# AlibabaResearch/efficientteacher

Measured on AMD Instinct MI355X. Metric: SSOD images/sec (teacher+student step) YOLOv5l 640px, higher is better.
Workload: dtype bf16

## Files before the change

efficientteacher_amd/csrc/conv.hip:

```cpp
#include "conv_host.h"

#ifndef ET_S1_NT
#define ET_S1_NT 1
#endif
#ifndef ET_GLDS_SHORTK_WGS
#define ET_GLDS_SHORTK_WGS 4
#endif


__device__ __forceinline__ void tap_lookup_uniform(const GatherGeom& g, int tap, int& dy, int& dx, int& wt) {
    const int ti = g.tapinfo[__builtin_amdgcn_readfirstlane(tap)];
    dy = (int)(signed char)(ti & 0xff);
    dx = (int)(signed char)((ti >> 8) & 0xff);
    wt = (ti >> 16) & 0xff;
}

__device__ __forceinline__ void tile_of_block(const GatherGeom& g, int& bx, int& by) {
    int id = blockIdx.x;
    if (g.nfast) {
        if (g.xcd_swz) {
            const int nb = gridDim.x, q = nb >> 3, r = nb & 7, xcd = id & 7, k = id >> 3;
            id = (xcd < r ? xcd * (q + 1) : r * (q + 1) + (xcd - r) * q) + k;
        }
        bx = id / g.ntn;
// ... 87 lines not shown
    constexpr int TN = BN / WN / 32, WCOLS = BN / WN, CVN = WCOLS / 8;
    const int l31 = lane & 31, hi = lane >> 5;
    const bool bnb = MODE == 1 ? false : ep.bn_y != nullptr;
    __syncthreads();
    float* const r0 = red + (wm * 2) * BN + wn * WCOLS;
    if (bnb) {
        const int scv = lane % CVN;
#pragma unroll
        for (int e = 0; e < 8; ++e)
            for (int m = CVN; m < 64; m <<= 1) { st.bs1[e] += __shfl_xor(st.bs1[e], m); st.bs2[e] += __shfl_xor(st.bs2[e], m); }
        if (lane < CVN) {
#pragma unroll
            for (int e = 0; e < 8; ++e) { r0[scv * 8 + e] = st.bs1[e]; r0[BN + scv * 8 + e] = st.bs2[e]; }
        }
    } else {
#pragma unroll
        for (int tn = 0; tn < TN; ++tn) {
            const float sv = st.ssum[tn] + __shfl_xor(st.ssum[tn], 32);
            const float qv = st.ssq[tn] + __shfl_xor(st.ssq[tn], 32);
            if (hi == 0) { r0[tn * 32 + l31] = sv; r0[BN + tn * 32 + l31] = qv; }
        }
    }
    __syncthreads();
    float* const dst = ep.stats + ((size_t)(blockIdx.x % ET_BN_SHARDS) * 2) * ep.stats_ld + n0;
    for (int i = tid; i < 2 * BN; i += 64 * WM * WN) {
        const int t = i / BN, c = i % BN;
        float v = 0.f;
#pragma unroll
        for (int w = 0; w < WM; ++w) v += red[(w * 2 + t) * BN + c];
        if (n0 + c < g.Cout) unsafeAtomicAdd(dst + (size_t)t * ep.stats_ld + c, v);
    }
}

template <typename T, int BM, int BN, int WM, int WN, int ACT, int SROWS = 32, int MODE = 0, bool DEFER = false, bool EPF = true>
__device__ __forceinline__ void conv_epilogue_act(f32x16 (&acc)[BM / WM / 32][BN / WN / 32], u32x4* lds_raw, T* __restrict__ Y,
                                                  const GatherGeom& g, const Epilogue& ep, int bx, int m0, int n0, int tid,
                                                  int lane, int wm, int wn, EpiSums<BN / WN / 32>& st) {
    constexpr int TM = BM / WM / 32, TN = BN / WN / 32;
    static_assert(SROWS == 32 || SROWS == 16, "slab rows");
    constexpr int NH = 32 / SROWS;
    using L = EpiLds<BM, BN, WM, WN, SROWS>;
    constexpr int WCOLS = L::WCOLS, SLD = L::SLD;
    constexpr int CVN = WCOLS / 8;
    constexpr int RPI = 64 / CVN;
    static_assert(RPI <= SROWS, "a store iteration covers at most one slab");
    const int l31 = lane & 31, hi = lane >> 5;
    const int wave = wm * WN + wn;
    float* const stg = (float*)lds_raw + wave * L::SLAB;
    float (&ssum)[TN] = st.ssum;
    float (&ssq)[TN] = st.ssq;
    float (&bs1)[8] = st.bs1;
    float (&bs2)[8] = st.bs2;
    const bool ident = (g.osy == 1 && g.osx == 1 && g.ooy == 0 && g.oox == 0 && g.QH == g.OH && g.QW == g.OW);
    float csc[TN], cbi[TN];
#pragma unroll
    for (int tn = 0; tn < TN; ++tn) {
        const int co = n0 + wn * WCOLS + tn * 32 + l31;
        const bool cok = co < g.Cout;
        if constexpr (DEFER) {
            csc[tn] = st.cst[co - n0];
            cbi[tn] = st.cst[st.cstride + co - n0];
        } else {
            csc[tn] = (ep.scale && cok) ? ep.scale[co] : 1.0f;
            cbi[tn] = (ep.bias && cok) ? ep.bias[co] : 0.0f;
        }
    }
    const int srow = lane / CVN, scv = lane % CVN;
    const int co = n0 + wn * WCOLS + scv * 8;
    const bool bnb = MODE == 1 ? false : ep.bn_y != nullptr;
    const void* const ep_res = MODE == 1 ? nullptr : ep.res;
    const bool ep_accumulate = MODE == 1 ? false : (bool)ep.accumulate;
    const bool lean = ident && !bnb && ep_res == nullptr && !ep_accumulate && m0 + (wm + 1) * (BM / WM) <= g.M && n0 + BN <= g.Cout;
    float bsc[8], bsh[8];
#pragma unroll
    for (int e = 0; e < 8; ++e) { bsc[e] = 1.f; bsh[e] = 0.f; }
    if (bnb && co + 8 <= g.Cout) {
#pragma unroll
        for (int e = 0; e < 8; ++e) {
            if constexpr (DEFER) { bsc[e] = st.cst[2 * st.cstride + co - n0 + e]; bsh[e] = st.cst[3 * st.cstride + co - n0 + e]; }
            else { bsc[e] = ep.bn_scale[co + e]; bsh[e] = ep.bn_shift[co + e]; }
        }
    }
    auto bn_bwd_sums = [&](const float (&dz8)[8], const float (&y8)[8]) {
        auto body = [&](auto act_tag) {
            constexpr int BACT = decltype(act_tag)::value;
#pragma unroll
            for (int e = 0; e < 8; ++e) {
                const float u = y8[e] * bsc[e] + bsh[e];
                float gact = 1.f;
                if constexpr (BACT == ACT_SILU) { const float sg = __builtin_amdgcn_rcpf(1.0f + __expf(-u)); gact = sg * (1.0f + u * (1.0f - sg)); }
                else if constexpr (BACT == ACT_RELU) gact = u > 0.f ? 1.f : 0.f;
                const float du = dz8[e] * gact;
                bs1[e] += du;
                bs2[e] += du * y8[e];
            }
        };
        if (ep.bn_act == ACT_SILU) body(std::integral_constant<int, ACT_SILU>{});
        else if (ep.bn_act == ACT_RELU) body(std::integral_constant<int, ACT_RELU>{});
        else body(std::integral_constant<int, ACT_NONE>{});
    };
    constexpr int NIT = SROWS / RPI;
    constexpr bool PF = EPF && sizeof(T) == 2 && MODE == 0;
    const bool pf_on = PF && !lean && (ep_res != nullptr || ep_accumulate || bnb);
    const bool pf_a_is_res = ep_res != nullptr;
    u32x4 pf_a[NIT], pf_b[NIT];
    auto pix_of = [&](int p) -> long long {
        if (ident) return p;
        const uint32_t t1 = fdiv((uint32_t)p, g.dQW), qx = p - t1 * g.QW;
        const uint32_t n = fdiv(t1, g.dQH), qy = t1 - n * g.QH;
        return ((long long)n * g.OH + (qy * g.osy + g.ooy)) * g.OW + (qx * g.osx + g.oox);
    };
#pragma unroll
    for (int tmh = 0; tmh < TM * NH; ++tmh) {
        const int tm = tmh / NH, hoff = (tmh % NH) * SROWS;
        if constexpr (PF) {
            if (pf_on) {
#pragma unroll
                for (int it = 0; it < NIT; ++it) {
                    const int p = m0 + wm * (BM / WM) + tm * 32 + hoff + it * RPI + srow;
                    if (p < g.M && co + 8 <= g.Cout) {
                        const long long pix = pix_of(p);
                        if (pf_a_is_res) pf_a[it] = *(const u32x4*)((const T*)ep_res + pix * ep.ldr + co);
                        else if (ep_accumulate) pf_a[it] = *(const u32x4*)(Y + pix * g.ldy + co);
                        if (bnb) pf_b[it] = *(const u32x4*)((const T*)ep.bn_y + pix * ep.ld_bn + co);
                    }
                }
            }
        }
#pragma unroll
        for (int rr = 0; rr < 16 / NH; ++rr) {
            const int r = (tmh % NH) * (16 / NH) + rr;
            const int row = (rr & 3) + 8 * (rr >> 2) + 4 * hi;
#pragma unroll
            for (int tn = 0; tn < TN; ++tn) {
                float v = acc[tm][tn][r];
                ssum[tn] += v;
                ssq[tn] += v * v;
                v = v * csc[tn] + cbi[tn];
                if constexpr (ACT == ACT_SILU) v = v * __builtin_amdgcn_rcpf(1.0f + __expf(-v));
                else if constexpr (ACT == ACT_RELU) v = fmaxf(v, 0.f);
                stg[row * SLD + tn * 32 + l31] = v;
            }
        }
        __builtin_amdgcn_s_waitcnt(0xC07F);
        __builtin_amdgcn_wave_barrier();
        if constexpr (sizeof(T) == 2) {
            if (lean) {
#pragma unroll
                for (int it = 0; it < SROWS / RPI; ++it) {
                    const int row = it * RPI + srow;
                    const long long p = m0 + wm * (BM / WM) + tm * 32 + hoff + row;
                    const float4 a = *(const float4*)(stg + row * SLD + scv * 8);
                    const float4 b = *(const float4*)(stg + row * SLD + scv * 8 + 4);
                    *(u32x4*)(Y + p * g.ldy + co) = mk4(et_lp<T>::pack(a.x, a.y), et_lp<T>::pack(a.z, a.w), et_lp<T>::pack(b.x, b.y), et_lp<T>::pack(b.z, b.w));
                }
                __builtin_amdgcn_s_waitcnt(0xC07F);
                __builtin_amdgcn_wave_barrier();
                continue;
            }
        }
#pragma unroll
        for (int it = 0; it < SROWS / RPI; ++it) {
            const int row = it * RPI + srow;
            const int p = m0 + wm * (BM / WM) + tm * 32 + hoff + row;
            if (p < g.M && co < g.Cout) {
                const long long pix = pix_of(p);
                float v[8];
                const float4 a = *(const float4*)(stg + row * SLD + scv * 8);
                const float4 b = *(const float4*)(stg + row * SLD + scv * 8 + 4);
                v[0] = a.x; v[1] = a.y; v[2] = a.z; v[3] = a.w; v[4] = b.x; v[5] = b.y; v[6] = b.z; v[7] = b.w;
                T* yp = Y + pix * g.ldy + co;
                if (co + 8 <= g.Cout) {
                    if constexpr (sizeof(T) == 2) {
                        if (ep_res) {
                            u32x4 rr;
// ... 31 lines not shown
                        }
                    } else {
                        if (ep_res) {
                            const float* rp = (const float*)ep_res + pix * ep.ldr + co;
                            const float4 r0 = *(const float4*)rp, r1 = *(const float4*)(rp + 4);
                            v[0] += r0.x; v[1] += r0.y; v[2] += r0.z; v[3] += r0.w; v[4] += r1.x; v[5] += r1.y; v[6] += r1.z; v[7] += r1.w;
                        }
                        if (ep_accumulate) {
                            const float4 r0 = *(const float4*)yp, r1 = *(const float4*)((const float*)yp + 4);
                            v[0] += r0.x; v[1] += r0.y; v[2] += r0.z; v[3] += r0.w; v[4] += r1.x; v[5] += r1.y; v[6] += r1.z; v[7] += r1.w;
                        }
                        *(float4*)yp = make_float4(v[0], v[1], v[2], v[3]);
                        *(float4*)((float*)yp + 4) = make_float4(v[4], v[5], v[6], v[7]);
                        if (bnb) {
                            const float* bp = (const float*)ep.bn_y + pix * ep.ld_bn + co;
                            const float4 y0 = *(const float4*)bp, y1 = *(const float4*)(bp + 4);
                            const float yv8[8] = {y0.x, y0.y, y0.z, y0.w, y1.x, y1.y, y1.z, y1.w};
                            bn_bwd_sums(v, yv8);
                        }
                    }
                } else {
                    for (int e = 0; e < 8 && co + e < g.Cout; ++e) {
                        float x = v[e];
                        if (ep_res) x += et_elem<T>::ld(((const T*)ep_res)[pix * ep.ldr + co + e]);
                        if (ep_accumulate) x += et_elem<T>::ld(yp[e]);
                        yp[e] = et_elem<T>::st(x);
                    }
                }
            }
        }
        __builtin_amdgcn_s_waitcnt(0xC07F);
        __builtin_amdgcn_wave_barrier();
    }
    if constexpr (!DEFER) {
        if (ep.stats) {
            constexpr int RPW = (BM / WM) / 64;
            static_assert((BM / WM) % 64 == 0, "wave tiles are whole 64-row blocks");
            if (ep.stats_ld) conv_stats_add_sharded_wg<BN, WN, WM, MODE>(st, g, ep, tid, lane, wm, wn, (float*)lds_raw, n0);
            else conv_epilogue_write_stats<BN, WN, MODE>(st, g, ep, n0, lane, wn, (m0 + wm * (BM / WM)) / 64, RPW - 1, (g.M + 63) / 64);
        }
    }
}

template <typename T, int BM, int BN, int WM, int WN, int SROWS = 32, int MODE = 0, bool DEFER = false, bool EPF = true>
__device__ __forceinline__ void conv_epilogue(f32x16 (&acc)[BM / WM / 32][BN / WN / 32], u32x4* lds_raw, T* __restrict__ Y,
                                              const GatherGeom& g, const Epilogue& ep, int bx, int m0, int n0, int tid,
                                              int lane, int wm, int wn, EpiSums<BN / WN / 32>& st) {
    if (ep.act == ACT_SILU) conv_epilogue_act<T, BM, BN, WM, WN, ACT_SILU, SROWS, MODE, DEFER, EPF>(acc, lds_raw, Y, g, ep, bx, m0, n0, tid, lane, wm, wn, st);
    else if (ep.act == ACT_RELU) conv_epilogue_act<T, BM, BN, WM, WN, ACT_RELU, SROWS, MODE, DEFER, EPF>(acc, lds_raw, Y, g, ep, bx, m0, n0, tid, lane, wm, wn, st);
    else conv_epilogue_act<T, BM, BN, WM, WN, ACT_NONE, SROWS, MODE, DEFER, EPF>(acc, lds_raw, Y, g, ep, bx, m0, n0, tid, lane, wm, wn, st);
}
template <typename T, int BM, int BN, int WM, int WN, bool EPF = true>
__device__ __forceinline__ void conv_epilogue(f32x16 (&acc)[BM / WM / 32][BN / WN / 32], u32x4* lds_raw, T* __restrict__ Y,
                                              const GatherGeom& g, const Epilogue& ep, int bx, int m0, int n0, int tid,
                                              int lane, int wm, int wn) {
    EpiSums<BN / WN / 32> st;
    st.clear();
    conv_epilogue<T, BM, BN, WM, WN, 32, 0, false, EPF>(acc, lds_raw, Y, g, ep, bx, m0, n0, tid, lane, wm, wn, st);
}

template <typename T, int BM, int BN, int WM, int WN, int BKV, bool UTAP>
__global__ __launch_bounds__(256) void conv_gemm_kernel(const T* __restrict__ X, const T* __restrict__ W,
                                                        T* __restrict__ Y, GatherGeom g, Epilogue ep) {
    constexpr int VEC = et_elem<T>::VEC;
    constexpr int TM = BM / WM / 32, TN = BN / WN / 32;
    constexpr int RPT = 256 / BKV;
    constexpr int RA = BM / RPT, RB = BN / RPT;
    constexpr int STAGE_VEC = (BM + BN) * BKV;
    constexpr int EPI_VEC = EpiLds<BM, BN, WM, WN>::VEC16;
    constexpr int LDS_VEC = 2 * STAGE_VEC > EPI_VEC ? 2 * STAGE_VEC : EPI_VEC;
    __shared__ __attribute__((aligned(16))) u32x4 lds_raw[LDS_VEC];
    u32x4* const lds0 = lds_raw;
    u32x4* const lds1 = lds_raw + STAGE_VEC;

    const int tid = threadIdx.x, lane = tid & 63, wave = tid >> 6;
    const int wm = wave / WN, wn = wave % WN;
    int bx, by;
    tile_of_block(g, bx, by);
    const int m0 = bx * BM, n0 = by * BN;
    const int lvec = tid % BKV, lrow = tid / BKV;

    int a_off[RA], a_iy[RA], a_ix[RA];
    bool a_ok[RA];
#pragma unroll
    for (int j = 0; j < RA; ++j) {
        const int p = m0 + lrow + j * RPT;
// ... 286 lines not shown
        const int P = P0 - 1 + rho;
        const uint32_t Pp = P < 0 ? 0 : P;
        const uint32_t yg = fdiv(Pp, g.dW1), xp = Pp - yg * W1;
        const uint32_t pix = yg * g.QW + xp;
        a_ok[q] = rho < CAP && P >= 0 && (int)xp < g.QW && pix < (uint32_t)g.M;
        const uint32_t ygc = a_ok[q] ? yg : 0;
        a_iy[q] = ygc - fdiv(ygc, g.dQH) * g.QH;
        a_off[q] = (a_ok[q] ? pix : 0) * g.ldx;
        a_lv[q] = lvec ^ lds_swz<BKV>(rho);
    }
    const int rowstep = g.IW * g.ldx;
    unsigned a_nokm = 0u;
    et_rsrc rsX, rsW;
    if constexpr (BUF) {
        rsX = et_make_rsrc((const char*)X - (size_t)rowstep * sizeof(T), (unsigned)(((size_t)g.N * g.IH * g.IW * g.ldx + rowstep) * sizeof(T)));
        rsW = et_make_rsrc(W, (unsigned)((size_t)g.Cout * g.TT * g.Cin * sizeof(T)));
#pragma unroll
        for (int q = 0; q < RA; ++q) {
            a_nokm |= ((a_iy[q] > 0 ? 0u : 1u) | (a_iy[q] + 1 < g.IH ? 0u : 4u)) << (3 * q);
            a_off[q] = a_ok[q] ? (int)((a_off[q] + a_lv[q] * VEC) * (int)sizeof(T)) : (int)0x80000000;
        }
    }
    int b_off[RB], b_lv[RB];
    bool b_ok[RB];
#pragma unroll
    for (int q = 0; q < RB; ++q) {
        const int rl = lrow + q * RPT;
        const int co = n0 + rl;
        b_ok[q] = co < g.Cout;
        b_off[q] = (b_ok[q] ? co : 0) * g.TT * g.Cin;
        b_lv[q] = lvec ^ lds_swz<BKV>(rl);
        if constexpr (BUF) b_off[q] = (int)((co * g.TT * g.Cin + b_lv[q] * VEC) * (int)sizeof(T));
    }
    int abase[TM][3];
#pragma unroll
    for (int tm = 0; tm < TM; ++tm) {
        const uint32_t p = m0 + wm * (BM / WM) + tm * 32 + (lane & 31);
        const uint32_t yg = fdiv(p, g.dQW);
        const int r0 = (int)(yg * W1 + (p - yg * g.QW)) - P0;
#pragma unroll
        for (int sft = 0; sft < 3; ++sft) abase[tm][sft] = ((r0 + sft) * BKV + ((lane >> 5) ^ lds_swz<BKV>(r0 + sft))) * 16;
    }

    f32x16 acc[TM][TN];
#pragma unroll
    for (int tm = 0; tm < TM; ++tm)
#pragma unroll
        for (int tn = 0; tn < TN; ++tn)
#pragma unroll
            for (int r = 0; r < 16; ++r) acc[tm][tn][r] = 0.f;

    const int sgn = g.dy[0] < 0 ? 1 : -1;
    auto stage_a = [&](u32x4* dst, int j, int cv_c) {
        u32x4* const wbase = dst + wave * 64;
        const int dy = sgn * (j - 1);
        const int roff = dy * g.IW * g.ldx + cv_c * VEC;
#pragma unroll
        for (int q = 0; q < RA; ++q) {
            if (q == RAF && wave >= XW) continue;
            if constexpr (BUF) {
                const unsigned bad = (a_nokm >> (3 * q + 1 + dy)) & 1u;
                et_bufdma16(rsX, (bad << 31) | (unsigned)a_off[q], (unsigned)(((dy + 1) * rowstep + cv_c * VEC) * (int)sizeof(T)), wbase + q * NT);
            } else {
                const bool ok = a_ok[q] && (unsigned)(a_iy[q] + dy) < (unsigned)g.IH;
                const T* src = ok ? X + (a_off[q] + roff + a_lv[q] * VEC) : ZERO;
                et_glds16(src, wbase + q * NT);
            }
        }
    };
    auto stage_b = [&](u32x4* dst, int tap, int cv_c) {
        u32x4* const wbase = dst + wave * 64;
        const int woff = tap * g.Cin + cv_c * VEC;
#pragma unroll
        for (int q = 0; q < RB; ++q) {
            if constexpr (BUF) {
                et_bufdma16(rsW, (unsigned)b_off[q], (unsigned)(woff * (int)sizeof(T)), wbase + q * NT);
            } else {
                const T* src = b_ok[q] ? W + (b_off[q] + woff + b_lv[q] * VEC) : ZERO;
                et_glds16(src, wbase + q * NT);
            }
        }
    };
    auto mma_step = [&](const u32x4* __restrict__ sa, const u32x4* __restrict__ sb, auto shift_tag) {
        constexpr int SFT = decltype(shift_tag)::value;
        const int l31 = lane & 31, gh = lane >> 5;
        u32x4 af[2][TM], bf[2][TN];
        auto fetch = [&](int kk, int set) {
#pragma unroll
            for (int tm = 0; tm < TM; ++tm) af[set][tm] = *(const u32x4*)((const char*)sa + (abase[tm][SFT] ^ (kk * 32)));
#pragma unroll
            for (int tn = 0; tn < TN; ++tn) {
                const int r = wn * (BN / WN) + tn * 32 + l31;
                bf[set][tn] = sb[r * BKV + ((kk * 2 + gh) ^ lds_swz<BKV>(r))];
            }
        };
        fetch(0, 0);
#pragma unroll
        for (int kk = 0; kk < BKV / 2; ++kk) {
            const int cur = kk & 1;
            if (kk + 1 < BKV / 2) {
                fetch(kk + 1, cur ^ 1);
                __builtin_amdgcn_sched_barrier(0);
            }
#pragma unroll
            for (int tm = 0; tm < TM; ++tm)
#pragma unroll
                for (int tn = 0; tn < TN; ++tn)
                    acc[tm][tn] = et_mfma32<T>(af[cur][tm], bf[cur][tn], acc[tm][tn]);
        }
    };

    const int nunits = 3 * (g.CV / BKV);
    stage_a(slotA, 0, 0);
    stage_b(slotB, sgn > 0 ? 0 : 2, 0);
    int j = 0, cv_u = 0, bs = 0;
#pragma unroll 1
    for (int u = 0; u < nunits; ++u) {
        const bool more_units = u + 1 < nunits;
        int nj = j + 1, ncv = cv_u;
        if (nj == 3) { nj = 0; ncv += BKV; }
        const u32x4* const sa = slotA + (u & 1) * A_VEC;
        auto step = [&](auto ktag) {
            constexpr int k = decltype(ktag)::value;
            if (k == 1 && more_units) {
                if (wave < XW) et_wait_vmem_le_lds_read_done<RA>(); else et_wait_vmem_le_lds_read_done<RAF>();
            } else {
                et_wait_vmem_lds_read_done();
            }
            __builtin_amdgcn_s_barrier();
            constexpr int kn = k < 2 ? k + 1 : 0;
            if (k < 2 || more_units) stage_b(slotB + (bs ^ 1) * B_VEC, (k < 2 ? j : nj) * 3 + (sgn > 0 ? kn : 2 - kn), k < 2 ? cv_u : ncv);
            if (k == 0 && more_units) stage_a(slotA + ((u + 1) & 1) * A_VEC, nj, ncv);
            mma_step(sa, slotB + bs * B_VEC, ktag);
            bs ^= 1;
        };
        step(std::integral_constant<int, 0>{});
        step(std::integral_constant<int, 1>{});
        step(std::integral_constant<int, 2>{});
        j = nj; cv_u = ncv;
    }
    __syncthreads();
// ... 33 lines not shown
    tile_of_block(g, bx, by);
    const int m0 = bx * BM, n0 = by * BN;
    const int lvec = tid & 7, lrow = tid >> 3;
    const int lv = lvec ^ lds_swz<BKV>(lrow);

    int a_off[2][2], a_iy[2][2], a_ix[2][2];
    unsigned a_okm = 0u, b_okm = 0u;
#pragma unroll
    for (int i = 0; i < 2; ++i)
#pragma unroll
        for (int jj = 0; jj < 2; ++jj) {
            const int p = m0 + jj * 128 + i * 64 + lrow;
            const bool ok = p < g.M;
            const uint32_t pp = ok ? p : 0;
            const uint32_t t1 = fdiv(pp, g.dQW), qx = pp - t1 * g.QW;
            const uint32_t n = fdiv(t1, g.dQH), qy = t1 - n * g.QH;
            a_iy[i][jj] = qy * g.isy;
            a_ix[i][jj] = qx * g.isx;
            a_off[i][jj] = ((n * g.IH + a_iy[i][jj]) * g.IW + a_ix[i][jj]) * g.ldx;
            a_okm |= ok ? (1u << (i * 2 + jj)) : 0u;
        }
    int b_off[2][2];
#pragma unroll
    for (int j = 0; j < 2; ++j)
#pragma unroll
        for (int jj = 0; jj < 2; ++jj) {
            const int r = jj * 64 + lrow;
            const int co = n0 + (r >> 5) * 64 + j * 32 + (r & 31);
            const bool ok = co < g.Cout;
            b_off[j][jj] = (ok ? co : 0) * g.TT * g.Cin;
            b_okm |= ok ? (1u << (j * 2 + jj)) : 0u;
        }

    f32x16 acc[4][2];
#pragma unroll
    for (int tm = 0; tm < 4; ++tm)
#pragma unroll
        for (int tn = 0; tn < 2; ++tn)
#pragma unroll
            for (int r = 0; r < 16; ++r) acc[tm][tn][r] = 0.f;

    const int nchunks = g.KV / BKV;
    int tap_u = 0, cv_u = 0;
    int ti_cur = g.tapinfo[0];
    int udy = 0, udx = 0, uwt = 0;
#define ET_PP_DECODE()                                                   \
    do {                                                                 \
        udy = (int)(signed char)(ti_cur & 0xff);                         \
        udx = (int)(signed char)((ti_cur >> 8) & 0xff);                  \
        uwt = (ti_cur >> 16) & 0xff;                                     \
    } while (0)
#define ET_PP_ADVANCE()                                                  \
    do {                                                                 \
        const int t2_ = tap_u + 1, c2_ = cv_u + BKV;                     \
        const bool wt_ = t2_ >= g.T, wc_ = c2_ >= g.CV;                  \
        const int ta_ = wt_ ? 0 : t2_, ca_ = wt_ ? c2_ : cv_u;           \
        const int cb_ = wc_ ? 0 : c2_, tb_ = wc_ ? t2_ : tap_u;          \
        tap_u = g.tap_inner ? ta_ : tb_;                                 \
        cv_u = g.tap_inner ? ca_ : cb_;                                  \
        ti_cur = g.tapinfo[__builtin_amdgcn_readfirstlane(tap_u < g.T ? tap_u : 0)]; \
    } while (0)
    auto stage_piece = [&](int k, int buf, int jj) {
        u32x4* const wbase = lds_raw + (2 * k + buf) * HALF_VEC + wave * 64;
        if (k < 2) {
            const int i = k;
            const int doff = (udy * g.IW + udx) * g.ldx + (cv_u + lv) * VEC;
            const bool ok = (bool)((a_okm >> (i * 2 + jj)) & 1u) & ((unsigned)(a_iy[i][jj] + udy) < (unsigned)g.IH) &
                            ((unsigned)(a_ix[i][jj] + udx) < (unsigned)g.IW);
            et_glds16(ok ? X + (a_off[i][jj] + doff) : ZERO, wbase + jj * 512);
        } else {
            const int j = k - 2;
            const int woff = uwt * g.Cin + (cv_u + lv) * VEC;
            const bool ok = (b_okm >> (j * 2 + jj)) & 1u;
            et_glds16(ok ? W + (b_off[j][jj] + woff) : ZERO, wbase + jj * 512);
        }
    };
    auto stage_a = [&](int i, int buf) { stage_piece(i, buf, 0); stage_piece(i, buf, 1); };
    auto stage_b = [&](int j, int buf) { stage_piece(2 + j, buf, 0); stage_piece(2 + j, buf, 1); };

    const int l31 = lane & 31, gk = lane >> 5;
    u32x4 af[2][4], bf[4];
    auto load_a = [&](int i, int buf) {
        const u32x4* sm = lds_raw + (2 * i + buf) * HALF_VEC;
#pragma unroll
        for (int t = 0; t < 2; ++t) {
            const int r = wm * 64 + t * 32 + l31;
#pragma unroll
            for (int kk = 0; kk < 4; ++kk) af[t][kk] = sm[r * BKV + ((kk * 2 + gk) ^ lds_swz<BKV>(r))];
        }
    };
    auto load_b = [&](int j, int buf) {
        const u32x4* sm = lds_raw + (2 * (2 + j) + buf) * HALF_VEC;
        const int r = wn * 32 + l31;
#pragma unroll
        for (int kk = 0; kk < 4; ++kk) bf[kk] = sm[r * BKV + ((kk * 2 + gk) ^ lds_swz<BKV>(r))];
    };
    auto mfma8 = [&](int i, int j, int sk, int sb) {
        __builtin_amdgcn_s_setprio(1);
        __builtin_amdgcn_sched_barrier(0);
#pragma unroll
        for (int kk = 0; kk < 4; ++kk)
#pragma unroll
            for (int t = 0; t < 2; ++t) {
                acc[2 * i + t][j] = et_mfma32<T>(af[t][kk], bf[kk], acc[2 * i + t][j]);
                const int n = kk * 2 + t;
                if (sk >= 0 && (n == 1 || n == 4)) {
                    __builtin_amdgcn_sched_barrier(0);
                    stage_piece(sk, sb, n == 1 ? 0 : 1);
                    __builtin_amdgcn_sched_barrier(0);
                }
            }
        __builtin_amdgcn_sched_barrier(0);
        __builtin_amdgcn_s_setprio(0);
    };

    ET_PP_DECODE();
    stage_a(0, 0); stage_b(0, 0); stage_b(1, 0); stage_a(1, 0);
    ET_PP_ADVANCE();
    et_wait_vmem();
    __builtin_amdgcn_s_barrier();
#define ET_PP_BAR() __builtin_amdgcn_s_barrier()
#define ET_PP_WAIT(n) et_wait_vmem_le_pp<n>()
    if (wm == 1) __builtin_amdgcn_s_barrier();

    auto chunk = [&](int buf, auto last_tag) {
        constexpr bool LAST = decltype(last_tag)::value;
        const int nb = buf ^ 1;
        if constexpr (!LAST) ET_PP_DECODE();
        load_a(0, buf); load_b(0, buf);
        ET_PP_WAIT(2);
        ET_PP_BAR();
        mfma8(0, 0, LAST ? -1 : 0, nb);
        ET_PP_BAR();
        load_b(1, buf);
        if constexpr (LAST) ET_PP_WAIT(0); else ET_PP_WAIT(2);
        ET_PP_BAR();
        mfma8(0, 1, LAST ? -1 : 2, nb);
        ET_PP_BAR();
        load_a(1, buf);
        ET_PP_BAR();
        mfma8(1, 1, LAST ? -1 : 3, nb);
        ET_PP_BAR();
        load_b(0, buf);
        if constexpr (!LAST) ET_PP_WAIT(2);
// ... 45 lines not shown
    const int P0 = (int)(yg0 * W1 + ((uint32_t)m0 - yg0 * g.QW));

    int a_off[NPIECE];
    unsigned a_okm = 0u, b_okm = 0u;
#pragma unroll
    for (int q = 0; q < NPIECE; ++q) {
        const int P = P0 - 1 + q * 64 + lrow;
        const uint32_t Pp = P < 0 ? 0 : P;
        const uint32_t yg = fdiv(Pp, g.dW1), xp = Pp - yg * W1;
        const uint32_t pix = yg * g.QW + xp;
        const bool ok = P >= 0 && (int)xp < g.QW && pix < (uint32_t)g.M;
        const uint32_t ygc = ok ? yg : 0;
        const int iy = ygc - fdiv(ygc, g.dQH) * g.QH;
        a_off[q] = (ok ? pix : 0) * g.ldx;
        a_okm |= ok ? ((iy > 0 ? 1u : 0u) | 2u | (iy + 1 < g.IH ? 4u : 0u)) << (3 * q) : 0u;
        if constexpr (BUF) a_off[q] = ok ? (int)((a_off[q] + lv * VEC) * (int)sizeof(T)) : (int)0x80000000;
    }
    const unsigned a_nokm = ~a_okm;
    const int co0 = n0 + (lrow >> 5) * 64 + (lrow & 31);
    const int wrow = g.TT * g.Cin;
    const int b_off0 = co0 * wrow;
    const int rowstep = g.IW * g.ldx;
    et_rsrc rsX, rsW;
    unsigned voffB = 0;
    if constexpr (BUF) {
        rsX = et_make_rsrc((const char*)X - (size_t)rowstep * sizeof(T), (unsigned)(((size_t)g.N * g.IH * g.IW * g.ldx + rowstep) * sizeof(T)));
        rsW = et_make_rsrc(W, (unsigned)((size_t)g.Cout * wrow * sizeof(T)));
        voffB = (unsigned)((b_off0 + lv * VEC) * (int)sizeof(T));
    }
#pragma unroll
    for (int j = 0; j < 2; ++j)
#pragma unroll
        for (int jj = 0; jj < 2; ++jj) b_okm |= (co0 + jj * 128 + j * 32 < g.Cout) ? (1u << (j * 2 + jj)) : 0u;
    const int l31 = lane & 31, gk = lane >> 5;
    int abase[2][2][3];
#pragma unroll
    for (int i = 0; i < 2; ++i)
#pragma unroll
        for (int t = 0; t < 2; ++t) {
            const uint32_t p = m0 + wm * 128 + i * 64 + t * 32 + l31;
            const uint32_t yg = fdiv(p, g.dQW);
            const int r0 = (int)(yg * W1 + (p - yg * g.QW)) - P0;
#pragma unroll
            for (int sft = 0; sft < 3; ++sft) abase[i][t][sft] = ((r0 + sft) * BKV + (gk ^ lds_swz<BKV>(r0 + sft))) * 16;
        }

    f32x16 acc[4][2];
#pragma unroll
    for (int tm = 0; tm < 4; ++tm)
#pragma unroll
        for (int tn = 0; tn < 2; ++tn)
#pragma unroll
            for (int r = 0; r < 16; ++r) acc[tm][tn][r] = 0.f;

    const int sgn = g.dy[0] < 0 ? 1 : -1;
    auto stage_a_piece = [&](int q, int ub, int j, int cv) {
        u32x4* const wbase = slotA + ub * A_VEC + q * 512 + wave * 64;
        const int dy = sgn * (j - 1);
        if constexpr (BUF) {
            const unsigned bad = (a_nokm >> (3 * q + 1 + dy)) & 1u;
            et_bufdma16(rsX, (bad << 31) | (unsigned)a_off[q], (unsigned)(((dy + 1) * rowstep + cv * VEC) * (int)sizeof(T)), wbase);
        } else {
            const bool ok = (a_okm >> (3 * q + 1 + dy)) & 1u;
            et_glds16(ok ? X + (a_off[q] + dy * g.IW * g.ldx + (cv + lv) * VEC) : ZERO, wbase);
        }
    };
    auto stage_b_piece = [&](int j, int b, int jj, int tap, int cv) {
        u32x4* const wbase = slotB + (2 * j + b) * HALF_VEC + wave * 64;
        if constexpr (BUF) {
            et_bufdma16(rsW, voffB, (unsigned)(((jj * 128 + j * 32) * wrow + tap * g.Cin + cv * VEC) * (int)sizeof(T)), wbase + jj * 512);
        } else {
            const bool ok = (b_okm >> (j * 2 + jj)) & 1u;
            et_glds16(ok ? W + (b_off0 + (jj * 128 + j * 32) * wrow + tap * g.Cin + (cv + lv) * VEC) : ZERO, wbase + jj * 512);
        }
    };

    u32x4 af[2][4], bf[4];
    auto load_a = [&](int i, int ub, auto shift_tag) {
        constexpr int SFT = decltype(shift_tag)::value;
        const char* sm = (const char*)(slotA + ub * A_VEC);
#pragma unroll
        for (int t = 0; t < 2; ++t)
#pragma unroll
            for (int kk = 0; kk < 4; ++kk) af[t][kk] = *(const u32x4*)(sm + (abase[i][t][SFT] ^ (kk * 32)));
    };
    auto load_b = [&](int j, int b) {
        const u32x4* sm = slotB + (2 * j + b) * HALF_VEC;
        const int r = wn * 32 + l31;
#pragma unroll
        for (int kk = 0; kk < 4; ++kk) bf[kk] = sm[r * BKV + ((kk * 2 + gk) ^ lds_swz<BKV>(r))];
    };
    auto mfma8 = [&](int i, int j, auto&& piece0, auto&& piece1) {
        __builtin_amdgcn_s_setprio(1);
        __builtin_amdgcn_sched_barrier(0);
#pragma unroll
        for (int kk = 0; kk < 4; ++kk)
#pragma unroll
            for (int t = 0; t < 2; ++t) {
                acc[2 * i + t][j] = et_mfma32<T>(af[t][kk], bf[kk], acc[2 * i + t][j]);
                const int n = kk * 2 + t;
                if (n == 1) { __builtin_amdgcn_sched_barrier(0); piece0(); __builtin_amdgcn_sched_barrier(0); }
                if (n == 4) { __builtin_amdgcn_sched_barrier(0); piece1(); __builtin_amdgcn_sched_barrier(0); }
            }
        __builtin_amdgcn_sched_barrier(0);
        __builtin_amdgcn_s_setprio(0);
    };
    auto nothing = [] {};

    const int nunits = 3 * (g.CV / BKV);
#pragma unroll
    for (int q = 0; q < NPIECE; ++q) stage_a_piece(q, 0, 0, 0);
#pragma unroll
    for (int j = 0; j < 2; ++j) { stage_b_piece(j, 0, 0, sgn > 0 ? 0 : 2, 0); stage_b_piece(j, 0, 1, sgn > 0 ? 0 : 2, 0); }
    et_wait_vmem();
    __builtin_amdgcn_s_barrier();
#define ET_PP_BAR() __builtin_amdgcn_s_barrier()
#define ET_PP_WAIT(n) et_wait_vmem_le_pp<n>()
    if (wm == 1) __builtin_amdgcn_s_barrier();

    int jrow = 0, cv_u = 0, bbuf = 0;
#pragma unroll 1
    for (int u = 0; u < nunits; ++u) {
        const bool more = u + 1 < nunits;
        int nj = jrow + 1, ncv = cv_u;
        if (nj == 3) { nj = 0; ncv += BKV; }
        const int ub = u & 1, nub = ub ^ 1;
        auto chunk = [&](auto ktag) {
            constexpr int k = decltype(ktag)::value;
            const bool stage_b = k < 2 || more;
            const int kn = k < 2 ? k + 1 : 0;
            const int ntap = (k < 2 ? jrow : nj) * 3 + (sgn > 0 ? kn : 2 - kn), nbcv = k < 2 ? cv_u : ncv;
            const int nb = bbuf ^ 1;
            const std::integral_constant<int, k> shift{};
            load_a(0, ub, shift); load_b(0, bbuf);
            if (k > 0 && more) ET_PP_WAIT(1); else ET_PP_WAIT(0);
            ET_PP_BAR();
// ... 266 lines not shown
```

efficientteacher_amd/csrc/conv_device.h:

```cpp
#pragma once
#include "et_device.h"
#include "../../include/et_hip.h"
#include <stdlib.h>
#include <stdio.h>
#include <string.h>
#include <type_traits>

typedef __attribute__((ext_vector_type(16))) float f32x16;
typedef __attribute__((ext_vector_type(8))) __bf16 bf16x8;
typedef __attribute__((ext_vector_type(8))) _Float16 f16x8;
typedef __attribute__((ext_vector_type(4))) unsigned int u32x4;
typedef short s16x4 __attribute__((ext_vector_type(4)));
typedef short s16x8 __attribute__((ext_vector_type(8)));
__device__ __forceinline__ u32x4 mk4(unsigned a, unsigned b, unsigned c, unsigned d) { u32x4 v = {a, b, c, d}; return v; }
__device__ __forceinline__ void et_pin_loaded(u32x4& v) {
#if defined(__HIP_DEVICE_COMPILE__)
    asm volatile("" : "+v"(v));
#endif
}

template <typename T, typename V> __device__ __forceinline__ f32x16 et_mfma32(const V a, const V b, const f32x16 c) {
    static_assert(sizeof(V) == 16, "8 x 16-bit operands");
    if constexpr (std::is_same<T, et_f16>::value)
        return __builtin_amdgcn_mfma_f32_32x32x16_f16(__builtin_bit_cast(f16x8, a), __builtin_bit_cast(f16x8, b), c, 0, 0, 0);
    else
        return __builtin_amdgcn_mfma_f32_32x32x16_bf16(__builtin_bit_cast(bf16x8, a), __builtin_bit_cast(bf16x8, b), c, 0, 0, 0);
}

#define CONV_MAX_TAPS 36
#define RS_A_ROWS(BM) ((BM) + 16)
#define PPRS_ROWS 320

struct FastDiv {
    uint32_t magic, shift, d;
};
static FastDiv make_fastdiv(uint32_t d) {
    FastDiv f;
    if (d == 0) d = 1;
    f.d = d;
    uint32_t s = 0;
    while ((1ull << s) < d) ++s;
    f.shift = s;
    f.magic = (uint32_t)((((1ull << 32) * ((1ull << s) - d)) / d) + 1);
    return f;
}
__device__ __forceinline__ uint32_t fdiv(uint32_t n, const FastDiv& f) {
    return (__umulhi(n, f.magic) + n) >> f.shift;
}

struct GatherGeom {
    int N, IH, IW, Cin, ldx;
    int QH, QW, M;
    int OH, OW, Cout, ldy;
    int isy, isx;
    int osy, osx, ooy, oox;
    int T, TT;
    int CV, KV;
    int tap_inner;
    int xcd_swz;
// ... 128 lines not shown
```

Measured before the change: 1321.

## Switch conv kernels from 32x32x16 to 16x16x32 MFMA with matching epilogue

```diff
diff --git a/efficientteacher_amd/csrc/conv.hip b/efficientteacher_amd/csrc/conv.hip
--- a/efficientteacher_amd/csrc/conv.hip
+++ b/efficientteacher_amd/csrc/conv.hip
@@ -143,12 +143,15 @@
     }
 }
 
-template <typename T, int BM, int BN, int WM, int WN, int ACT, int SROWS = 32, int MODE = 0, bool DEFER = false, bool EPF = true>
-__device__ __forceinline__ void conv_epilogue_act(f32x16 (&acc)[BM / WM / 32][BN / WN / 32], u32x4* lds_raw, T* __restrict__ Y,
+template <typename T, int BM, int BN, int WM, int WN, int ACT, int SROWS = 32, int MODE = 0, bool DEFER = false, bool EPF = true, typename ACC>
+__device__ __forceinline__ void conv_epilogue_act(ACC& acc, u32x4* lds_raw, T* __restrict__ Y,
                                                   const GatherGeom& g, const Epilogue& ep, int bx, int m0, int n0, int tid,
                                                   int lane, int wm, int wn, EpiSums<BN / WN / 32>& st) {
     constexpr int TM = BM / WM / 32, TN = BN / WN / 32;
-    static_assert(SROWS == 32 || SROWS == 16, "slab rows");
+    constexpr bool M16 = std::is_same<ACC, f32x4[TM][TN][2][2]>::value;
+    static_assert(M16 || std::is_same<ACC, f32x16[TM][TN]>::value, "accumulator form");
+    constexpr int NCI = M16 ? 2 : 1;
+    static_assert(SROWS == 32 || (SROWS == 16 && !M16), "slab rows");
     constexpr int NH = 32 / SROWS;
     using L = EpiLds<BM, BN, WM, WN, SROWS>;
     constexpr int WCOLS = L::WCOLS, SLD = L::SLD;
@@ -163,19 +166,24 @@
     float (&bs1)[8] = st.bs1;
     float (&bs2)[8] = st.bs2;
     const bool ident = (g.osy == 1 && g.osx == 1 && g.ooy == 0 && g.oox == 0 && g.QH == g.OH && g.QW == g.OW);
-    float csc[TN], cbi[TN];
-#pragma unroll
-    for (int tn = 0; tn < TN; ++tn) {
-        const int co = n0 + wn * WCOLS + tn * 32 + l31;
-        const bool cok = co < g.Cout;
-        if constexpr (DEFER) {
-            csc[tn] = st.cst[co - n0];
-            cbi[tn] = st.cst[st.cstride + co - n0];
-        } else {
-            csc[tn] = (ep.scale && cok) ? ep.scale[co] : 1.0f;
-            cbi[tn] = (ep.bias && cok) ? ep.bias[co] : 0.0f;
-        }
-    }
+    const int lcol = M16 ? (lane & 15) : l31;
+    float csc[TN][NCI], cbi[TN][NCI];
+    float s16[TN][NCI], q16[TN][NCI];
+#pragma unroll
+    for (int tn = 0; tn < TN; ++tn)
+#pragma unroll
+        for (int ci = 0; ci < NCI; ++ci) {
+            const int co = n0 + wn * WCOLS + tn * 32 + ci * 16 + lcol;
+            const bool cok = co < g.Cout;
+            if constexpr (DEFER) {
+                csc[tn][ci] = st.cst[co - n0];
+                cbi[tn][ci] = st.cst[st.cstride + co - n0];
+            } else {
+                csc[tn][ci] = (ep.scale && cok) ? ep.scale[co] : 1.0f;
+                cbi[tn][ci] = (ep.bias && cok) ? ep.bias[co] : 0.0f;
+            }
+            s16[tn][ci] = 0.f; q16[tn][ci] = 0.f;
+        }
     const int srow = lane / CVN, scv = lane % CVN;
     const int co = n0 + wn * WCOLS + scv * 8;
     const bool bnb = MODE == 1 ? false : ep.bn_y != nullptr;
@@ -239,19 +247,28 @@
             }
         }
 #pragma unroll
-        for (int rr = 0; rr < 16 / NH; ++rr) {
+        for (int rr = 0; rr < (M16 ? 8 : 16) / NH; ++rr) {
             const int r = (tmh % NH) * (16 / NH) + rr;
-            const int row = (rr & 3) + 8 * (rr >> 2) + 4 * hi;
-#pragma unroll
-            for (int tn = 0; tn < TN; ++tn) {
-                float v = acc[tm][tn][r];
-                ssum[tn] += v;
-                ssq[tn] += v * v;
-                v = v * csc[tn] + cbi[tn];
-                if constexpr (ACT == ACT_SILU) v = v * __builtin_amdgcn_rcpf(1.0f + __expf(-v));
-                else if constexpr (ACT == ACT_RELU) v = fmaxf(v, 0.f);
-                stg[row * SLD + tn * 32 + l31] = v;
-            }
+            const int row = M16 ? 16 * (rr >> 2) + 4 * (lane >> 4) + (rr & 3) : (rr & 3) + 8 * (rr >> 2) + 4 * hi;
+#pragma unroll
+            for (int tn = 0; tn < TN; ++tn)
+#pragma unroll
+                for (int ci = 0; ci < NCI; ++ci) {
+                    float v;
+                    if constexpr (M16) {
+                        v = acc[tm][tn][rr >> 2][ci][rr & 3];
+                        s16[tn][ci] += v;
+                        q16[tn][ci] += v * v;
+                    } else {
+                        v = acc[tm][tn][r];
+                        ssum[tn] += v;
+                        ssq[tn] += v * v;
+                    }
+                    v = v * csc[tn][ci] + cbi[tn][ci];
+                    if constexpr (ACT == ACT_SILU) v = v * __builtin_amdgcn_rcpf(1.0f + __expf(-v));
+                    else if constexpr (ACT == ACT_RELU) v = fmaxf(v, 0.f);
+                    stg[row * SLD + tn * 32 + ci * 16 + lcol] = v;
+                }
         }
         __builtin_amdgcn_s_waitcnt(0xC07F);
         __builtin_amdgcn_wave_barrier();
@@ -349,6 +366,14 @@
         __builtin_amdgcn_s_waitcnt(0xC07F);
         __builtin_amdgcn_wave_barrier();
     }
+    if constexpr (M16) {
+        const bool up = (lane >> 4) & 1;
+#pragma unroll
+        for (int tn = 0; tn < TN; ++tn) {
+            ssum[tn] += (up ? s16[tn][1] : s16[tn][0]) + __shfl_xor(up ? s16[tn][0] : s16[tn][1], 16);
+            ssq[tn] += (up ? q16[tn][1] : q16[tn][0]) + __shfl_xor(up ? q16[tn][0] : q16[tn][1], 16);
+        }
+    }
     if constexpr (!DEFER) {
         if (ep.stats) {
             constexpr int RPW = (BM / WM) / 64;
@@ -359,16 +384,16 @@
     }
 }
 
-template <typename T, int BM, int BN, int WM, int WN, int SROWS = 32, int MODE = 0, bool DEFER = false, bool EPF = true>
-__device__ __forceinline__ void conv_epilogue(f32x16 (&acc)[BM / WM / 32][BN / WN / 32], u32x4* lds_raw, T* __restrict__ Y,
+template <typename T, int BM, int BN, int WM, int WN, int SROWS = 32, int MODE = 0, bool DEFER = false, bool EPF = true, typename ACC>
+__device__ __forceinline__ void conv_epilogue(ACC& acc, u32x4* lds_raw, T* __restrict__ Y,
                                               const GatherGeom& g, const Epilogue& ep, int bx, int m0, int n0, int tid,
                                               int lane, int wm, int wn, EpiSums<BN / WN / 32>& st) {
     if (ep.act == ACT_SILU) conv_epilogue_act<T, BM, BN, WM, WN, ACT_SILU, SROWS, MODE, DEFER, EPF>(acc, lds_raw, Y, g, ep, bx, m0, n0, tid, lane, wm, wn, st);
     else if (ep.act == ACT_RELU) conv_epilogue_act<T, BM, BN, WM, WN, ACT_RELU, SROWS, MODE, DEFER, EPF>(acc, lds_raw, Y, g, ep, bx, m0, n0, tid, lane, wm, wn, st);
     else conv_epilogue_act<T, BM, BN, WM, WN, ACT_NONE, SROWS, MODE, DEFER, EPF>(acc, lds_raw, Y, g, ep, bx, m0, n0, tid, lane, wm, wn, st);
 }
-template <typename T, int BM, int BN, int WM, int WN, bool EPF = true>
-__device__ __forceinline__ void conv_epilogue(f32x16 (&acc)[BM / WM / 32][BN / WN / 32], u32x4* lds_raw, T* __restrict__ Y,
+template <typename T, int BM, int BN, int WM, int WN, bool EPF = true, typename ACC>
+__device__ __forceinline__ void conv_epilogue(ACC& acc, u32x4* lds_raw, T* __restrict__ Y,
                                               const GatherGeom& g, const Epilogue& ep, int bx, int m0, int n0, int tid,
                                               int lane, int wm, int wn) {
     EpiSums<BN / WN / 32> st;
@@ -721,23 +746,25 @@
         b_lv[q] = lvec ^ lds_swz<BKV>(rl);
         if constexpr (BUF) b_off[q] = (int)((co * g.TT * g.Cin + b_lv[q] * VEC) * (int)sizeof(T));
     }
-    int abase[TM][3];
-#pragma unroll
-    for (int tm = 0; tm < TM; ++tm) {
-        const uint32_t p = m0 + wm * (BM / WM) + tm * 32 + (lane & 31);
+    int abase[2 * TM][3];
+#pragma unroll
+    for (int ts = 0; ts < 2 * TM; ++ts) {
+        const uint32_t p = m0 + wm * (BM / WM) + ts * 16 + (lane & 15);
         const uint32_t yg = fdiv(p, g.dQW);
         const int r0 = (int)(yg * W1 + (p - yg * g.QW)) - P0;
 #pragma unroll
-        for (int sft = 0; sft < 3; ++sft) abase[tm][sft] = ((r0 + sft) * BKV + ((lane >> 5) ^ lds_swz<BKV>(r0 + sft))) * 16;
-    }
-
-    f32x16 acc[TM][TN];
+        for (int sft = 0; sft < 3; ++sft) abase[ts][sft] = ((r0 + sft) * BKV + ((lane >> 4) ^ lds_swz<BKV>(r0 + sft))) * 16;
+    }
+
+    f32x4 acc[TM][TN][2][2];
 #pragma unroll
     for (int tm = 0; tm < TM; ++tm)
 #pragma unroll
         for (int tn = 0; tn < TN; ++tn)
 #pragma unroll
-            for (int r = 0; r < 16; ++r) acc[tm][tn][r] = 0.f;
+            for (int q = 0; q < 4; ++q)
+#pragma unroll
+                for (int r = 0; r < 4; ++r) acc[tm][tn][q >> 1][q & 1][r] = 0.f;
 
     const int sgn = g.dy[0] < 0 ? 1 : -1;
     auto stage_a = [&](u32x4* dst, int j, int cv_c) {
@@ -772,30 +799,38 @@
     };
     auto mma_step = [&](const u32x4* __restrict__ sa, const u32x4* __restrict__ sb, auto shift_tag) {
         constexpr int SFT = decltype(shift_tag)::value;
-        const int l31 = lane & 31, gh = lane >> 5;
-        u32x4 af[2][TM], bf[2][TN];
-        auto fetch = [&](int kk, int set) {
-#pragma unroll
-            for (int tm = 0; tm < TM; ++tm) af[set][tm] = *(const u32x4*)((const char*)sa + (abase[tm][SFT] ^ (kk * 32)));
-#pragma unroll
-            for (int tn = 0; tn < TN; ++tn) {
-                const int r = wn * (BN / WN) + tn * 32 + l31;
-                bf[set][tn] = sb[r * BKV + ((kk * 2 + gh) ^ lds_swz<BKV>(r))];
-            }
+        const int l15 = lane & 15, gq = lane >> 4;
+        u32x4 af[2][TM], bf[2][TN][2];
+        auto fetch_a = [&](int stg) {
+#pragma unroll
+            for (int tm = 0; tm < TM; ++tm) af[stg & 1][tm] = *(const u32x4*)((const char*)sa + (abase[2 * tm + (stg & 1)][SFT] ^ ((stg >> 1) * 64)));
         };
-        fetch(0, 0);
-#pragma unroll
-        for (int kk = 0; kk < BKV / 2; ++kk) {
-            const int cur = kk & 1;
-            if (kk + 1 < BKV / 2) {
-                fetch(kk + 1, cur ^ 1);
+        auto fetch_b = [&](int kk) {
+#pragma unroll
+            for (int tn = 0; tn < TN; ++tn)
+#pragma unroll
+                for (int ci = 0; ci < 2; ++ci) {
+                    const int r = wn * (BN / WN) + tn * 32 + ci * 16 + l15;
+                    bf[kk & 1][tn][ci] = sb[r * BKV + ((kk * 4 + gq) ^ lds_swz<BKV>(r))];
+                }
+        };
+        fetch_a(0);
+        fetch_b(0);
+#pragma unroll
+        for (int stg = 0; stg < BKV / 2; ++stg) {
+            const int kk = stg >> 1, ri = stg & 1;
+            if (stg + 1 < BKV / 2) {
+                fetch_a(stg + 1);
+                if (ri == 1) fetch_b(kk + 1);
                 __builtin_amdgcn_sched_barrier(0);
             }
 #pragma unroll
             for (int tm = 0; tm < TM; ++tm)
 #pragma unroll
                 for (int tn = 0; tn < TN; ++tn)
-                    acc[tm][tn] = et_mfma32<T>(af[cur][tm], bf[cur][tn], acc[tm][tn]);
+#pragma unroll
+                    for (int ci = 0; ci < 2; ++ci)
+                        acc[tm][tn][ri][ci] = et_mfma16<T>(af[ri][tm], bf[kk & 1][tn][ci], acc[tm][tn][ri][ci]);
         }
     };
 
@@ -895,13 +930,15 @@
             b_okm |= ok ? (1u << (j * 2 + jj)) : 0u;
         }
 
-    f32x16 acc[4][2];
+    f32x4 acc[4][2][2][2];
 #pragma unroll
     for (int tm = 0; tm < 4; ++tm)
 #pragma unroll
         for (int tn = 0; tn < 2; ++tn)
 #pragma unroll
-            for (int r = 0; r < 16; ++r) acc[tm][tn][r] = 0.f;
+            for (int q = 0; q < 4; ++q)
+#pragma unroll
+                for (int r = 0; r < 4; ++r) acc[tm][tn][q >> 1][q & 1][r] = 0.f;
 
     const int nchunks = g.KV / BKV;
     int tap_u = 0, cv_u = 0;
@@ -941,38 +978,43 @@
     auto stage_a = [&](int i, int buf) { stage_piece(i, buf, 0); stage_piece(i, buf, 1); };
     auto stage_b = [&](int j, int buf) { stage_piece(2 + j, buf, 0); stage_piece(2 + j, buf, 1); };
 
-    const int l31 = lane & 31, gk = lane >> 5;
-    u32x4 af[2][4], bf[4];
+    const int l15 = lane & 15, gk = lane >> 4;
+    u32x4 af[4][2], bf[2][2];
     auto load_a = [&](int i, int buf) {
         const u32x4* sm = lds_raw + (2 * i + buf) * HALF_VEC;
 #pragma unroll
-        for (int t = 0; t < 2; ++t) {
-            const int r = wm * 64 + t * 32 + l31;
-#pragma unroll
-            for (int kk = 0; kk < 4; ++kk) af[t][kk] = sm[r * BKV + ((kk * 2 + gk) ^ lds_swz<BKV>(r))];
+        for (int ts = 0; ts < 4; ++ts) {
+            const int r = wm * 64 + ts * 16 + l15;
+#pragma unroll
+            for (int kk = 0; kk < 2; ++kk) af[ts][kk] = sm[r * BKV + ((kk * 4 + gk) ^ lds_swz<BKV>(r))];
         }
     };
     auto load_b = [&](int j, int buf) {
         const u32x4* sm = lds_raw + (2 * (2 + j) + buf) * HALF_VEC;
-        const int r = wn * 32 + l31;
-#pragma unroll
-        for (int kk = 0; kk < 4; ++kk) bf[kk] = sm[r * BKV + ((kk * 2 + gk) ^ lds_swz<BKV>(r))];
+#pragma unroll
+        for (int ci = 0; ci < 2; ++ci) {
+            const int r = wn * 32 + ci * 16 + l15;
+#pragma unroll
+            for (int kk = 0; kk < 2; ++kk) bf[ci][kk] = sm[r * BKV + ((kk * 4 + gk) ^ lds_swz<BKV>(r))];
+        }
     };
     auto mfma8 = [&](int i, int j, int sk, int sb) {
         __builtin_amdgcn_s_setprio(1);
         __builtin_amdgcn_sched_barrier(0);
 #pragma unroll
-        for (int kk = 0; kk < 4; ++kk)
-#pragma unroll
-            for (int t = 0; t < 2; ++t) {
-                acc[2 * i + t][j] = et_mfma32<T>(af[t][kk], bf[kk], acc[2 * i + t][j]);
-                const int n = kk * 2 + t;
-                if (sk >= 0 && (n == 1 || n == 4)) {
-                    __builtin_amdgcn_sched_barrier(0);
-                    stage_piece(sk, sb, n == 1 ? 0 : 1);
-                    __builtin_amdgcn_sched_barrier(0);
+        for (int kk = 0; kk < 2; ++kk)
+#pragma unroll
+            for (int ts = 0; ts < 4; ++ts)
+#pragma unroll
+                for (int ci = 0; ci < 2; ++ci) {
+                    acc[2 * i + (ts >> 1)][j][ts & 1][ci] = et_mfma16<T>(af[ts][kk], bf[ci][kk], acc[2 * i + (ts >> 1)][j][ts & 1][ci]);
+                    const int n = (kk * 4 + ts) * 2 + ci;
+                    if (sk >= 0 && (n == 3 || n == 9)) {
+                        __builtin_amdgcn_sched_barrier(0);
+                        stage_piece(sk, sb, n == 3 ? 0 : 1);
+                        __builtin_amdgcn_sched_barrier(0);
+                    }
                 }
-            }
         __builtin_amdgcn_sched_barrier(0);
         __builtin_amdgcn_s_setprio(0);
     };
@@ -1084,26 +1126,43 @@
     for (int j = 0; j < 2; ++j)
 #pragma unroll
         for (int jj = 0; jj < 2; ++jj) b_okm |= (co0 + jj * 128 + j * 32 < g.Cout) ? (1u << (j * 2 + jj)) : 0u;
-    const int l31 = lane & 31, gk = lane >> 5;
-    int abase[2][2][3];
+    const int l15 = lane & 15, gk = lane >> 4;
+    int abase[2][4][BUF ? 3 : 2];
 #pragma unroll
     for (int i = 0; i < 2; ++i)
 #pragma unroll
-        for (int t = 0; t < 2; ++t) {
-            const uint32_t p = m0 + wm * 128 + i * 64 + t * 32 + l31;
+        for (int ts = 0; ts < 4; ++ts) {
+            const uint32_t p = m0 + wm * 128 + i * 64 + ts * 16 + l15;
             const uint32_t yg = fdiv(p, g.dQW);
             const int r0 = (int)(yg * W1 + (p - yg * g.QW)) - P0;
-#pragma unroll
-            for (int sft = 0; sft < 3; ++sft) abase[i][t][sft] = ((r0 + sft) * BKV + (gk ^ lds_swz<BKV>(r0 + sft))) * 16;
-        }
-
-    f32x16 acc[4][2];
+            int o[3];
+#pragma unroll
+            for (int sft = 0; sft < 3; ++sft) o[sft] = ((r0 + sft) * BKV + (gk ^ lds_swz<BKV>(r0 + sft))) * 16;
+            if constexpr (BUF) { abase[i][ts][0] = o[0]; abase[i][ts][1] = o[1]; abase[i][ts][2] = o[2]; }
+            else { abase[i][ts][0] = o[0] | (o[1] << 16); abase[i][ts][1] = o[2]; }
+        }
+    static_assert(A_VEC * 16 <= (1 << 16), "a fragment offset fits 16 bits");
+    auto a_addr = [&](int i, int ts, int sft) -> int {
+        if constexpr (BUF) return abase[i][ts][sft];
+        else if (sft == 2) return abase[i][ts][1];
+        else {
+            unsigned pk = (unsigned)abase[i][ts][0];
+#if defined(__HIP_DEVICE_COMPILE__)
+            asm volatile("" : "+v"(pk));
+#endif
+            return sft == 0 ? (int)(pk & 0xffffu) : (int)(pk >> 16);
+        }
+    };
+
+    f32x4 acc[4][2][2][2];
 #pragma unroll
     for (int tm = 0; tm < 4; ++tm)
 #pragma unroll
         for (int tn = 0; tn < 2; ++tn)
 #pragma unroll
-            for (int r = 0; r < 16; ++r) acc[tm][tn][r] = 0.f;
+            for (int q = 0; q < 4; ++q)
+#pragma unroll
+                for (int r = 0; r < 4; ++r) acc[tm][tn][q >> 1][q & 1][r] = 0.f;
 
     const int sgn = g.dy[0] < 0 ? 1 : -1;
     auto stage_a_piece = [&](int q, int ub, int j, int cv) {
@@ -1127,33 +1186,38 @@
         }
     };
 
-    u32x4 af[2][4], bf[4];
+    u32x4 af[4][2], bf[2][2];
     auto load_a = [&](int i, int ub, auto shift_tag) {
         constexpr int SFT = decltype(shift_tag)::value;
         const char* sm = (const char*)(slotA + ub * A_VEC);
 #pragma unroll
-        for (int t = 0; t < 2; ++t)
-#pragma unroll
-            for (int kk = 0; kk < 4; ++kk) af[t][kk] = *(const u32x4*)(sm + (abase[i][t][SFT] ^ (kk * 32)));
+        for (int ts = 0; ts < 4; ++ts)
+#pragma unroll
+            for (int kk = 0; kk < 2; ++kk) af[ts][kk] = *(const u32x4*)(sm + (a_addr(i, ts, SFT) ^ (kk * 64)));
     };
     auto load_b = [&](int j, int b) {
         const u32x4* sm = slotB + (2 * j + b) * HALF_VEC;
-        const int r = wn * 32 + l31;
-#pragma unroll
-        for (int kk = 0; kk < 4; ++kk) bf[kk] = sm[r * BKV + ((kk * 2 + gk) ^ lds_swz<BKV>(r))];
+#pragma unroll
+        for (int ci = 0; ci < 2; ++ci) {
+            const int r = wn * 32 + ci * 16 + l15;
+#pragma unroll
+            for (int kk = 0; kk < 2; ++kk) bf[ci][kk] = sm[r * BKV + ((kk * 4 + gk) ^ lds_swz<BKV>(r))];
+        }
     };
     auto mfma8 = [&](int i, int j, auto&& piece0, auto&& piece1) {
         __builtin_amdgcn_s_setprio(1);
         __builtin_amdgcn_sched_barrier(0);
 #pragma unroll
-        for (int kk = 0; kk < 4; ++kk)
-#pragma unroll
-            for (int t = 0; t < 2; ++t) {
-                acc[2 * i + t][j] = et_mfma32<T>(af[t][kk], bf[kk], acc[2 * i + t][j]);
-                const int n = kk * 2 + t;
-                if (n == 1) { __builtin_amdgcn_sched_barrier(0); piece0(); __builtin_amdgcn_sched_barrier(0); }
-                if (n == 4) { __builtin_amdgcn_sched_barrier(0); piece1(); __builtin_amdgcn_sched_barrier(0); }
-            }
+        for (int kk = 0; kk < 2; ++kk)
+#pragma unroll
+            for (int ts = 0; ts < 4; ++ts)
+#pragma unroll
+                for (int ci = 0; ci < 2; ++ci) {
+                    acc[2 * i + (ts >> 1)][j][ts & 1][ci] = et_mfma16<T>(af[ts][kk], bf[ci][kk], acc[2 * i + (ts >> 1)][j][ts & 1][ci]);
+                    const int n = (kk * 4 + ts) * 2 + ci;
+                    if (n == 3) { __builtin_amdgcn_sched_barrier(0); piece0(); __builtin_amdgcn_sched_barrier(0); }
+                    if (n == 9) { __builtin_amdgcn_sched_barrier(0); piece1(); __builtin_amdgcn_sched_barrier(0); }
+                }
         __builtin_amdgcn_sched_barrier(0);
         __builtin_amdgcn_s_setprio(0);
     };
diff --git a/efficientteacher_amd/csrc/conv_device.h b/efficientteacher_amd/csrc/conv_device.h
--- a/efficientteacher_amd/csrc/conv_device.h
+++ b/efficientteacher_amd/csrc/conv_device.h
@@ -25,6 +25,18 @@
         return __builtin_amdgcn_mfma_f32_32x32x16_f16(__builtin_bit_cast(f16x8, a), __builtin_bit_cast(f16x8, b), c, 0, 0, 0);
     else
         return __builtin_amdgcn_mfma_f32_32x32x16_bf16(__builtin_bit_cast(bf16x8, a), __builtin_bit_cast(bf16x8, b), c, 0, 0, 0);
+}
+
+typedef __attribute__((ext_vector_type(4))) float f32x4;
+#if defined(__builtin_amdgcn_mfma_f32_16x16x32_bf16) && !defined(__builtin_amdgcn_mfma_f32_16x16x32_f16)
+#define __builtin_amdgcn_mfma_f32_16x16x32_f16(a, b, c, x, y, z) emu_mfma16<8>((a), (b), (c), emu_cvt_f16())
+#endif
+template <typename T, typename V> __device__ __forceinline__ f32x4 et_mfma16(const V a, const V b, const f32x4 c) {
+    static_assert(sizeof(V) == 16, "8 x 16-bit operands");
+    if constexpr (std::is_same<T, et_f16>::value)
+        return __builtin_amdgcn_mfma_f32_16x16x32_f16(__builtin_bit_cast(f16x8, a), __builtin_bit_cast(f16x8, b), c, 0, 0, 0);
+    else
+        return __builtin_amdgcn_mfma_f32_16x16x32_bf16(__builtin_bit_cast(bf16x8, a), __builtin_bit_cast(bf16x8, b), c, 0, 0, 0);
 }
 
 #define CONV_MAX_TAPS 36
```

After: 1326, median of 6. About the same (+0.4%).
